# mrvollger/rustybam

Measured on AMD Instinct MI355X. Metric: CIGAR-ops/s, liftover over 100 kb sliding windows (whole pass, inputs resident in HBM), higher is better.
Workload: dtype u32

## Files before the change

### include/rustybam_amd.h

```cpp
#ifndef RUSTYBAM_AMD_H
#define RUSTYBAM_AMD_H

#include <stddef.h>
#include <stdint.h>

#ifdef __cplusplus
extern "C" {
#endif

#define RB_ABI_VERSION 1

enum rb_op { RB_OP_M = 0, RB_OP_I = 1, RB_OP_D = 2, RB_OP_N = 3, RB_OP_S = 4, RB_OP_H = 5, RB_OP_P = 6, RB_OP_EQ = 7, RB_OP_X = 8,
             RB_OP_CONT = 14  };

typedef enum rb_error {
    RB_OK = 0,
    RB_E_INVALID = -1,
    RB_E_NO_DEVICE = -2,
    RB_E_HIP = -3,
    RB_E_CAPACITY = -4,
    RB_E_NOMEM = -5
} rb_error;

typedef enum rb_status {
// ... 51 lines not shown
} rb_norm_row;

typedef struct rb_hit_row {
    uint32_t rec, win;
    uint16_t status, flags;
    uint32_t out_n;
    uint64_t t_st, t_en, q_st, q_en;
    uint32_t nmatch, aln_len;
    uint64_t out_off;
} rb_hit_row;

typedef struct rb_pair_row {
    uint64_t split_idx;
    int32_t split_score;
    uint32_t status;
    uint64_t t_st[2], t_en[2], q_st[2], q_en[2];
    uint32_t nmatch[2], aln_len[2];
    uint64_t out_off[2];
    uint32_t out_n[2];
    uint64_t _pad;
} rb_pair_row;

typedef struct rb_counters {
    uint64_t n_hits;
    uint64_t out_ops_needed;
    uint64_t out_ops_used;
    uint64_t n_generic;
    uint32_t overflow;
    uint32_t phase[5];
    uint32_t brk_scratch_short;
    uint32_t redo_two_walk;
} rb_counters;

enum { RB_TEXT_OK = 0, RB_TEXT_BAD = 1 , RB_TEXT_TOO_LONG = 2 ,
       RB_TEXT_UNUSUAL = 3  };

typedef struct rb_batch_view {
    uint64_t n_rec, n_ops;
    const uint32_t *ops;
    const uint64_t *op_off;
    const uint64_t *t_st, *t_en, *q_st, *q_en;
    const uint8_t *strand;
    const uint32_t *contig;
} rb_batch_view;

typedef struct rb_windows_view {
    uint64_t n_win;
    const uint32_t *contig;
    const uint64_t *st, *en;
} rb_windows_view;

typedef struct rb_ctx rb_ctx;
typedef struct rb_plan rb_plan;

int rb_abi_version(void);
int rb_device_count(void);
int rb_ctx_create(int device, void *hip_stream, rb_ctx **out);
void rb_ctx_destroy(rb_ctx *ctx);
const char *rb_ctx_last_error(const rb_ctx *ctx);
int rb_ctx_sync(rb_ctx *ctx);
void *rb_ctx_stream(rb_ctx *ctx);
int rb_ctx_set_timing(rb_ctx *ctx, int enabled);
int rb_ctx_get_timing(rb_ctx *ctx, double *ms_out, int cap, int *n_out);

int rb_dev_alloc(rb_ctx *ctx, size_t bytes, void **dev_ptr);
int rb_dev_free(rb_ctx *ctx, void *dev_ptr);
int rb_dev_alloc_mode(rb_ctx *ctx, const void *dev_ptr);
int rb_dev_release(rb_ctx *ctx, void *dev_ptr);
int rb_dev_cache_trim(rb_ctx *ctx, uint64_t keep_bytes);
int rb_dev_alloc_stats(rb_ctx *ctx, uint64_t out[5]);
int rb_dev_upload(rb_ctx *ctx, void *dev_dst, const void *host_src, size_t bytes);
int rb_dev_download(rb_ctx *ctx, void *host_dst, const void *dev_src, size_t bytes);
int rb_dev_memset(rb_ctx *ctx, void *dev_dst, int value, size_t bytes);

int rb_dev_scan_records(rb_ctx *ctx, const rb_batch_view *batch, rb_reduce_row *reduce_rows, rb_norm_row *norm_rows);
int rb_ctx_scan_route(rb_ctx *ctx, uint64_t out[2]);

int rb_plan_create(rb_ctx *ctx, uint64_t n_rec, const uint64_t *op_off_host, const uint32_t *contig_host,
                   uint64_t n_win, const uint32_t *w_contig_host, const uint64_t *w_st_host, const uint64_t *w_en_host,
                   rb_plan **out);
void rb_plan_destroy(rb_plan *plan);
int64_t rb_plan_tiles_host(uint64_t n_rec, const uint64_t *op_off_host, uint64_t short_max, uint32_t *sched_out, uint32_t *tiles_out,
                           uint64_t tiles_cap, uint64_t *n_long_out);
size_t rb_plan_workspace_bytes(const rb_plan *plan, uint64_t rows_cap);
size_t rb_plan_diag_stamps_offset(const rb_plan *plan, uint64_t rows_cap);
uint64_t rb_plan_out_capacity(const rb_plan *plan, int for_break);

int rb_dev_liftover(rb_ctx *ctx, const rb_plan *plan, const rb_batch_view *batch, const rb_norm_row *norm_rows,
                    int bsearch_policy, void *workspace, rb_hit_row *rows, uint64_t rows_cap, uint32_t *out_ops,
                    uint64_t out_cap, rb_counters *counters);

size_t rb_largest_scratch_bytes(uint64_t n_keys);
int rb_dev_largest(rb_ctx *ctx, const rb_hit_row *rows, uint64_t n_rows, const uint32_t *win_key, const uint32_t *rec_key,
                   uint64_t n_keys, uint64_t *sel, uint64_t *out, void *scratch);

int rb_dev_break(rb_ctx *ctx, const rb_plan *plan, const rb_batch_view *batch, const rb_norm_row *norm_rows,
                 uint32_t max_size, int bsearch_policy, void *workspace, rb_hit_row *rows, uint64_t rows_cap,
                 uint32_t *out_ops, uint64_t out_cap, rb_counters *counters);

int rb_dev_swap(rb_ctx *ctx, const rb_batch_view *batch, uint32_t *out_ops);

enum { RB_TRIM_IN_PLACE = 256 };
int rb_dev_overlap_split(rb_ctx *ctx, const rb_batch_view *batch, const rb_norm_row *norm_rows, uint64_t n_pairs,
                         const uint32_t *left, const uint32_t *right, const uint64_t *pair_out_off, int match_score,
                         int diff_score, int indel_score, int bsearch_policy, rb_pair_row *rows, uint32_t *out_ops);

int rb_dev_trim_reserve(rb_ctx *ctx, uint64_t n_pairs);

int rb_dev_apply_pairs(rb_ctx *ctx, uint64_t n_pairs, const uint32_t *left, const uint32_t *right, const rb_pair_row *rows,
                       uint64_t *op_off, rb_norm_row *norm_rows);

typedef struct rb_trim_pass {
    uint64_t n_pairs, n_deferred, ops_end;
    uint32_t bad_status, _pad;
    uint64_t _reserved[4];
} rb_trim_pass;
size_t rb_trim_select_scratch_bytes(uint64_t n_groups);
int rb_dev_trim_select(rb_ctx *ctx, uint64_t n_rec, uint64_t n_groups, const uint32_t *order, const uint64_t *grp_off,
                       const rb_norm_row *norm_rows, uint64_t out_base, uint8_t *contained, uint32_t *left, uint32_t *right,
                       uint64_t *pair_out_off, rb_trim_pass *pass, void *scratch);
int rb_dev_trim_check(rb_ctx *ctx, uint64_t n_pairs, const rb_pair_row *rows, rb_trim_pass *pass);
int rb_dev_gather_records(rb_ctx *ctx, uint64_t n_rec, const uint32_t *ops, const uint64_t *op_off, const rb_norm_row *norm_rows,
                          uint64_t *new_op_off, uint32_t *new_ops, void *scratch);

int rb_host_scan_records(rb_ctx *ctx, uint64_t n_rec, const uint32_t *ops, const uint64_t *op_off,
                         const uint64_t *t_st, const uint64_t *t_en, const uint64_t *q_st, const uint64_t *q_en,
                         const uint8_t *strand, rb_reduce_row *reduce_rows, rb_norm_row *norm_rows);
int rb_host_liftover(rb_ctx *ctx, uint64_t n_rec, const uint32_t *ops, const uint64_t *op_off, const uint64_t *t_st,
                     const uint64_t *t_en, const uint64_t *q_st, const uint64_t *q_en, const uint8_t *strand,
                     const uint32_t *contig, uint64_t n_win, const uint32_t *w_contig, const uint64_t *w_st,
                     const uint64_t *w_en, int bsearch_policy, rb_norm_row *norm_rows_out ,
                     rb_hit_row **rows, uint64_t *n_rows, uint32_t **out_ops, uint64_t *n_out, rb_counters *counters);
int rb_host_break(rb_ctx *ctx, uint64_t n_rec, const uint32_t *ops, const uint64_t *op_off, const uint64_t *t_st,
                  const uint64_t *t_en, const uint64_t *q_st, const uint64_t *q_en, const uint8_t *strand,
                  uint32_t max_size, int bsearch_policy, rb_norm_row *norm_rows_out, rb_hit_row **rows,
                  uint64_t *n_rows, uint32_t **out_ops, uint64_t *n_out, rb_counters *counters);
int rb_host_swap(rb_ctx *ctx, uint64_t n_rec, const uint32_t *ops, const uint64_t *op_off, const uint8_t *strand,
                 uint32_t *out_ops);
int rb_host_overlap_split(rb_ctx *ctx, uint64_t n_rec, const uint32_t *ops, const uint64_t *op_off, const uint64_t *t_st,
                          const uint64_t *t_en, const uint64_t *q_st, const uint64_t *q_en, const uint8_t *strand,
                          uint64_t n_pairs, const uint32_t *left, const uint32_t *right, int match_score, int diff_score,
                          int indel_score, int bsearch_policy, rb_pair_row *rows, uint32_t **out_ops, uint64_t *n_out);
void rb_host_free(void *p);

size_t rb_text_scratch_bytes(uint64_t n);
int rb_dev_parse_cigars(rb_ctx *ctx, const uint8_t *text, const uint64_t *text_off, const uint64_t *text_end, uint64_t n_rec,
                        uint64_t *op_off, uint32_t *ops, uint64_t ops_cap, uint8_t *status, void *scratch);
int rb_dev_format_cigars(rb_ctx *ctx, const uint32_t *ops, const uint32_t *ops_alt, uint64_t n_items, const uint64_t *first,
                         const uint32_t *count, const uint32_t *first_len, const uint32_t *last_len, uint64_t *text_off, uint8_t *text,
                         uint64_t text_cap, void *scratch);
int rb_host_parse_cigars(rb_ctx *ctx, const uint8_t *text, const uint64_t *text_off, const uint64_t *text_end, uint64_t n_rec,
                         uint64_t *op_off, uint32_t **ops, uint8_t *status);
int rb_host_format_cigars(rb_ctx *ctx, const uint32_t *ops, uint64_t n_ops, uint64_t n_items, const uint64_t *first, const uint32_t *count,
                          const uint32_t *first_len, const uint32_t *last_len, uint64_t *text_off, uint8_t **text);
int rb_host_liftover_text(rb_ctx *ctx, uint64_t n_rec, const uint8_t *text, uint64_t text_bytes, const uint64_t *cig_off,
                          const uint64_t *cig_end, const uint64_t *t_st, const uint64_t *t_en, const uint64_t *q_st, const uint64_t *q_en,
                          const uint8_t *strand, const uint32_t *contig, uint64_t n_win, const uint32_t *w_contig, const uint64_t *w_st,
                          const uint64_t *w_en, int bsearch_policy, uint8_t *cig_status, rb_reduce_row *reduce_out, rb_norm_row *norm_out,
                          rb_hit_row **rows, uint64_t *n_rows, uint64_t **row_text_off, uint8_t **row_text, rb_counters *counters);
int rb_host_liftover_largest_text(rb_ctx *ctx, uint64_t n_rec, const uint8_t *text, uint64_t text_bytes, const uint64_t *cig_off,
                                  const uint64_t *cig_end, const uint64_t *t_st, const uint64_t *t_en, const uint64_t *q_st, const uint64_t *q_en,
                                  const uint8_t *strand, const uint32_t *contig, uint64_t n_win, const uint32_t *w_contig, const uint64_t *w_st,
                                  const uint64_t *w_en, int bsearch_policy, uint8_t *cig_status, rb_reduce_row *reduce_out, rb_norm_row *norm_out,
                                  rb_hit_row **rows, uint64_t *n_rows, uint64_t **row_text_off, uint8_t **row_text, rb_counters *counters,
                                  const uint32_t *win_key, uint64_t n_keys, uint32_t inside_key, int *declined);
int rb_host_break_text(rb_ctx *ctx, uint64_t n_rec, const uint8_t *text, uint64_t text_bytes, const uint64_t *cig_off,
// ... 52 lines not shown
```

### rustybam_amd/capi.py

```python
import ctypes as C
import os
import sys
import re

import numpy as np

HERE = os.path.dirname(os.path.abspath(__file__))
ROOT = os.path.dirname(HERE)
HEADER = os.path.join(ROOT, "include", "rustybam_amd.h")

BSEARCH_MODERN, BSEARCH_LEGACY, LIFT_EARLY_EXIT, LIFT_DESCRIPTORS, LIFT_FUSED_SCAN = 0, 1, 16, 32, 64
TRIM_IN_PLACE = 256
LIFT_OP_STARTS = 1 << 20
BREAK_ONE_WALK = 128
HIT_INSIDE, HIT_GENERIC, HIT_DESCRIPTOR = 1, 2, 4
NF_COVERED = 0x80000000
RD_OK, RD_FILTERED, RD_BAD_CIGAR, RD_SEQ_SHORT = 0, 1, 2, 3

REDUCE_DT = np.dtype(
    [("t_bases", "<u8"), ("q_bases", "<u8"), ("nmatch", "<u4"), ("aln_len", "<u4"), ("equal", "<u4"),
     ("diff", "<u4"), ("ins", "<u4"), ("del", "<u4"), ("matches", "<u4"), ("ins_events", "<u4"),
     ("del_events", "<u4"), ("id_by_all", "<f4"), ("id_by_events", "<f4"), ("id_by_matches", "<f4"),
     ("status", "<u4"), ("flags", "<u4")])
NORM_DT = np.dtype(
# ... 397 lines not shown
        end = None if text_end is None else _arr(text_end, np.uint64)
        op_off = np.zeros(n + 1, np.uint64)
        status = np.zeros(max(n, 1), np.uint8)
        out = C.c_void_p()
        self._chk(self.L.rb_host_parse_cigars(self.ctx, _p(text), _p(text_off), _p(end) if end is not None else None,
                                              C.c_uint64(n), _p(op_off), C.byref(out), _p(status)), "rb_host_parse_cigars")
        n_ops = int(op_off[n])
        if n_ops:
            ops = np.frombuffer((C.c_char * (n_ops * 4)).from_address(out.value), dtype=np.uint32).copy()
        else:
            ops = np.zeros(0, np.uint32)
        self.L.rb_host_free(out)
        return op_off, ops, status[:n]

    def format_cigars(self, ops, first, count, first_len=None, last_len=None):
        ops, first, count = _arr(ops, np.uint32), _arr(first, np.uint64), _arr(count, np.uint32)
        n = len(first)
        fl = None if first_len is None else _arr(first_len, np.uint32)
        ll = None if last_len is None else _arr(last_len, np.uint32)
        toff = np.zeros(n + 1, np.uint64)
        out = C.c_void_p()
        src = np.concatenate([ops, np.zeros(4, np.uint32)])
        self._chk(self.L.rb_host_format_cigars(self.ctx, _p(src), C.c_uint64(len(ops)), C.c_uint64(n), _p(first), _p(count),
                                               _p(fl) if fl is not None else None, _p(ll) if ll is not None else None, _p(toff),
                                               C.byref(out)), "rb_host_format_cigars")
        nb = int(toff[n])
        text = bytes((C.c_char * nb).from_address(out.value)) if nb else b""
        self.L.rb_host_free(out)
        return toff, text


    def nucfreq_workspace_bytes(self, n_reads, n_regions, n_pos):
        f = self.L.rb_nucfreq_workspace_bytes
        f.restype = C.c_size_t
        return int(f(C.c_uint64(n_reads), C.c_uint64(n_regions), C.c_uint64(n_pos)))

    def dev_nucfreq(self, n_reads, ops, op_off, seq, seq_off, l_seq, tid, pos, flag, n_regions, rg_tid, rg_st, rg_en, out_off, n_pos,
                    counts, status, counters, ws, ws_bytes):
        class View(C.Structure):
            _fields_ = [("n_reads", C.c_uint64), ("ops", C.c_void_p), ("op_off", C.c_void_p), ("seq", C.c_void_p), ("seq_off", C.c_void_p),
                        ("l_seq", C.c_void_p), ("tid", C.c_void_p), ("pos", C.c_void_p), ("flag", C.c_void_p)]
        v = View(n_reads, ops, op_off, seq, seq_off, l_seq, tid, pos, flag)
        self._chk(self.L.rb_dev_nucfreq(self.ctx, C.byref(v), C.c_uint64(n_regions), C.c_void_p(rg_tid), C.c_void_p(rg_st), C.c_void_p(rg_en),
                                        C.c_void_p(out_off), C.c_uint64(n_pos), C.c_void_p(counts), C.c_void_p(status), C.c_void_p(counters),
                                        C.c_void_p(ws), C.c_size_t(ws_bytes)), "rb_dev_nucfreq")

    def nucfreq(self, tid, pos, flag, op_off, ops, l_seq, seq_off, seq, rg_tid, rg_st, rg_en):
        tid, pos, flag = _arr(tid, np.int32), _arr(pos, np.int64), _arr(flag, np.uint32)
        op_off, ops = _arr(op_off, np.uint64), np.concatenate([_arr(ops, np.uint32), np.zeros(4, np.uint32)])
        l_seq, seq_off = _arr(l_seq, np.uint32), _arr(seq_off, np.uint64)
        seq = np.concatenate([_arr(seq, np.uint8), np.zeros(32, np.uint8)])
        rg_tid, rg_st, rg_en = _arr(rg_tid, np.int32), _arr(rg_st, np.uint64), _arr(rg_en, np.uint64)
        n, nr = len(tid), len(rg_tid)
        n_pos = int((rg_en.astype(np.int64) - rg_st.astype(np.int64)).sum()) if nr else 0

        class View(C.Structure):
            _fields_ = [("n_reads", C.c_uint64), ("ops", C.c_void_p), ("op_off", C.c_void_p), ("seq", C.c_void_p), ("seq_off", C.c_void_p),
                        ("l_seq", C.c_void_p), ("tid", C.c_void_p), ("pos", C.c_void_p), ("flag", C.c_void_p)]
        v = View(n, ops.ctypes.data, op_off.ctypes.data, seq.ctypes.data, seq_off.ctypes.data, l_seq.ctypes.data, tid.ctypes.data,
                 pos.ctypes.data, flag.ctypes.data)
        counts = np.zeros((max(n_pos, 1), 4), np.uint32)
        status = np.zeros(max(n, 1), np.uint32)
        ctr = np.zeros(6, np.uint64)
        self._chk(self.L.rb_host_nucfreq(self.ctx, C.byref(v), C.c_uint64(nr), _p(rg_tid), _p(rg_st), _p(rg_en), _p(counts), _p(status),
                                         _p(ctr)), "rb_host_nucfreq")
        return counts[:n_pos], status[:n], dict(max_depth=int(ctr[0]), n_covered=int(ctr[1]), n_bad=int(ctr[2]), unsorted=int(ctr[3]),
                                                    n_dropped=int(ctr[4]), cap_overflow=int(ctr[5]))


def synth_n_ops(seed, first_record, n_rec, lo, hi):
    L = lib()
    return np.array([L.rb_synth_n_ops(seed, first_record + i, lo, hi) for i in range(n_rec)], dtype=np.uint64)


def synth_fill_ops_host(seed, first_record, op_off):
    L = lib()
    op_off = _arr(op_off, np.uint64)
    ops = np.zeros(int(op_off[-1]), np.uint32)
    L.rb_synth_fill_ops_host(C.c_uint64(seed), C.c_uint64(first_record), C.c_uint64(len(op_off) - 1), _p(op_off),
                             _p(ops))
    return ops


class DevBuf:

    def __init__(self, eng, torch, n, dtype, device=None, placed_tries=1, score=None):
        self.eng, self.n, self.dtype = eng, int(n), dtype
        self.item = torch.empty(0, dtype=dtype).element_size()
        self.placement = None

        def take():
            if placed_tries > 1:
                ptr, ms, kept = eng.dev_alloc_placed(max(self.n * self.item, 256), placed_tries, score)
                self.placement = {("launch_ms" if score else "sweep_ms"): ms, "kept": kept}
                return ptr
            return eng.dev_alloc(max(self.n * self.item, 256))
        try:
            self.ptr = take()
        except Exception:
            torch.cuda.empty_cache()
            self.ptr = take()
        self.chunked = eng.L.rb_dev_alloc_mode(eng.ctx, C.c_void_p(self.ptr)) == 1
        self.__cuda_array_interface__ = {"shape": (self.n * self.item,), "typestr": "|u1", "data": (self.ptr, False), "version": 3}
        try:
            self.t = torch.as_tensor(self, device=device if device is not None else "cuda").view(dtype)
            if device is not None and self.t.device != torch.device(device):
                raise RuntimeError(f"the buffer was taken for {self.t.device}, not {device}")
        except Exception:
            self.t = None
            eng.dev_free(self.ptr)
            self.ptr = 0
            raise

    def free(self):
        if self.ptr:
            self.t = None
            self.eng.dev_free(self.ptr)
            self.ptr = 0

    def release(self):
        if self.ptr:
            self.t = None
            self.eng.dev_release(self.ptr)
            self.ptr = 0
```

### rustybam_amd/csrc/capi.hip

```cpp
#include <hip/hip_runtime.h>
#include <sys/mman.h>

#include <algorithm>
#include <cstdarg>
#include <cstdio>
#include <cstdlib>
#include <cstring>
#include <ctime>
#include <numeric>
#include <string>
#include <thread>
#include <vector>
#include <chrono>
#include <map>
#include <mutex>

#include "../../include/rustybam_amd.h"
#include "rb_lift.h"
#include "rb_trim.h"
#include "rb_launch.h"

#ifndef RB_SCAN_ROWS_MEAN_MAX
#define RB_SCAN_ROWS_MEAN_MAX 1536
#endif
#ifndef RB_SHORT_MAX_DEFAULT
#define RB_SHORT_MAX_DEFAULT 2048
#endif

#define RB_MAX_ARENA 256

#define RB_TIMING_RING 256
__global__ __launch_bounds__(256) void rb_k_fill_bytes(uint8_t *dst, uint32_t v4, size_t n) {
    const uintptr_t a = (uintptr_t)dst;
    const size_t head = n < 16 ? n : (size_t)((16 - (a & 15)) & 15);
    const size_t body = (n - head) / 16;
    const size_t tail0 = head + body * 16;
    const size_t i = (size_t)blockIdx.x * blockDim.x + threadIdx.x, stride = (size_t)gridDim.x * blockDim.x;
    for (size_t k = i; k < body; k += stride) *reinterpret_cast<uint4 *>(dst + head + k * 16) = make_uint4(v4, v4, v4, v4);
    if (i < head) dst[i] = (uint8_t)v4;
    if (i < n - tail0) dst[tail0 + i] = (uint8_t)v4;
}
extern "C" hipError_t rb_fill_async(void *dst, int value, size_t bytes, hipStream_t stream) {
    if (!bytes) return hipSuccess;
    const uint32_t b = (uint32_t)value & 255u, v4 = b | (b << 8) | (b << 16) | (b << 24);
    const size_t groups = bytes / 16 + 1;
    const unsigned blocks = (unsigned)std::min<size_t>((groups + 255) / 256, 65536);
    hipLaunchKernelGGL(rb_k_fill_bytes, dim3(blocks ? blocks : 1), dim3(256), 0, stream, (uint8_t *)dst, v4, bytes);
    return hipGetLastError();
}

struct rb_ctx {
    int device = -1;
    hipStream_t stream = nullptr;
    bool own_stream = false;
    std::string err;
    bool timing = false;
    std::vector<hipEvent_t> ev_a, ev_b;
    uint64_t timed_calls = 0;
    void *trim_scratch = nullptr;
    uint32_t trim_scratch_blocks = 0;
    void *trim_pend = nullptr;
    uint64_t trim_pend_cap = 0;
    void *scan_list = nullptr;
    uint64_t scan_list_cap = 0;
    uint64_t scan_rows_n = 0;
    void *pin[2] = {nullptr, nullptr};
    hipEvent_t pin_ev[2] = {nullptr, nullptr};
    bool pin_busy[2] = {false, false};
    unsigned pin_next = 0;
    uint64_t alloc_fallbacks = 0;
    struct cached_buf { void *p; size_t bytes; bool placed; };
    std::vector<cached_buf> cache;
    size_t cache_bytes = 0;
};
#define RB_PIN_CHUNK ((size_t)32 << 20)
#define RB_PIN_MIN ((size_t)8 << 20)

struct rb_plan {
    rb_ctx *ctx = nullptr;
    uint64_t n_rec = 0, n_win = 0, n_ops = 0;
    uint32_t n_contig = 0;
    uint32_t depth = 0;
    uint32_t *sched = nullptr, *slot_of = nullptr, *canon_pos = nullptr, *w_orig = nullptr, *ident = nullptr;
    uint64_t *w_st = nullptr, *w_en = nullptr, *wo_st = nullptr, *wo_en = nullptr, *cw_off = nullptr;
    uint8_t *cw_mono = nullptr;
    uint32_t *tiles = nullptr;
    uint32_t n_tiles = 0, stream_end = 0;
};

static int fail(rb_ctx *ctx, int code, const char *fmt, ...) {
    if (ctx) {
        char buf[512];
        va_list ap;
        va_start(ap, fmt);
        vsnprintf(buf, sizeof buf, fmt, ap);
        va_end(ap);
        ctx->err = buf;
    }
    return code;
}
#define HIPCHK(ctx, call)                                                                             \
    do {                                                                                              \
        hipError_t e_ = (call);                                                                       \
        if (e_ != hipSuccess) return fail((ctx), RB_E_HIP, "%s: %s", #call, hipGetErrorString(e_)); \
    } while (0)

extern "C" int rb_abi_version(void) { return RB_ABI_VERSION; }

extern "C" int rb_device_count(void) {
    int n = 0;
    if (hipGetDeviceCount(&n) != hipSuccess) return 0;
    return n;
}

extern "C" int rb_ctx_create(int device, void *hip_stream, rb_ctx **out) {
    if (!out) return RB_E_INVALID;
    *out = nullptr;
    int n = 0;
    if (hipGetDeviceCount(&n) != hipSuccess || n <= 0 || device < 0 || device >= n) return RB_E_NO_DEVICE;
    hipDeviceProp_t prop;
    if (hipGetDeviceProperties(&prop, device) != hipSuccess) return RB_E_NO_DEVICE;
    if (strncmp(prop.gcnArchName, "gfx950", 6) != 0) {
        fprintf(stderr, "rustybam_amd: device %d is %s; this library only carries gfx950 (MI355X) code objects\n", device, prop.gcnArchName);
        return RB_E_NO_DEVICE;
    }
    if (hipSetDevice(device) != hipSuccess) return RB_E_NO_DEVICE;
    rb_ctx *c = new rb_ctx();
    c->device = device;
    if (hip_stream) {
        c->stream = (hipStream_t)hip_stream;
    } else {
        if (hipStreamCreateWithFlags(&c->stream, hipStreamNonBlocking) != hipSuccess) {
            delete c;
            return RB_E_HIP;
        }
        c->own_stream = true;
    }
    *out = c;
    return RB_OK;
}
extern "C" void rb_ctx_destroy(rb_ctx *ctx) {
    if (!ctx) return;
    for (auto e : ctx->ev_a) hipEventDestroy(e);
    for (auto e : ctx->ev_b) hipEventDestroy(e);
    for (int k = 0; k < 2; k++) {
        if (ctx->pin[k]) hipHostFree(ctx->pin[k]);
        if (ctx->pin_ev[k]) hipEventDestroy(ctx->pin_ev[k]);
    }
    if (ctx->trim_scratch) hipFree(ctx->trim_scratch);
    if (ctx->trim_pend) hipFree(ctx->trim_pend);
    if (ctx->scan_list) hipFree(ctx->scan_list);
    (void)rb_dev_cache_trim(ctx, 0);
    if (ctx->own_stream) hipStreamDestroy(ctx->stream);
    delete ctx;
}
extern "C" const char *rb_ctx_last_error(const rb_ctx *ctx) { return ctx ? ctx->err.c_str() : "no context"; }
extern "C" int rb_ctx_sync(rb_ctx *ctx) {
    if (!ctx) return RB_E_INVALID;
    HIPCHK(ctx, hipStreamSynchronize(ctx->stream));
    return RB_OK;
}
extern "C" void *rb_ctx_stream(rb_ctx *ctx) { return ctx ? (void *)ctx->stream : nullptr; }

extern "C" int rb_ctx_set_timing(rb_ctx *ctx, int enabled) {
    if (!ctx) return RB_E_INVALID;
    if (enabled && ctx->ev_a.empty()) {
        ctx->ev_a.resize(RB_TIMING_RING);
        ctx->ev_b.resize(RB_TIMING_RING);
        for (int i = 0; i < RB_TIMING_RING; i++) {
            HIPCHK(ctx, hipEventCreate(&ctx->ev_a[i]));
            HIPCHK(ctx, hipEventCreate(&ctx->ev_b[i]));
        }
    }
    ctx->timing = enabled != 0;
    ctx->timed_calls = 0;
    return RB_OK;
}
extern "C" int rb_ctx_get_timing(rb_ctx *ctx, double *ms_out, int cap, int *n_out) {
    if (!ctx || !ms_out || !n_out) return RB_E_INVALID;
    HIPCHK(ctx, hipStreamSynchronize(ctx->stream));
    const uint64_t have = ctx->timed_calls < RB_TIMING_RING ? ctx->timed_calls : RB_TIMING_RING;
    int n = 0;
    for (uint64_t k = 0; k < have && n < cap; k++) {
        const uint64_t call = ctx->timed_calls - have + k;
        const size_t slot = (size_t)(call % RB_TIMING_RING);
        float ms = 0;
        HIPCHK(ctx, hipEventElapsedTime(&ms, ctx->ev_a[slot], ctx->ev_b[slot]));
        ms_out[n++] = ms;
    }
    *n_out = n;
    return RB_OK;
}

struct rb_vmm_alloc {
    size_t bytes, chunk;
    std::vector<hipMemGenericAllocationHandle_t> handles;
    bool placed = false;
};
static std::map<void *, rb_vmm_alloc> g_vmm;
static std::mutex g_vmm_mu;
static size_t g_va_live = 0, g_va_retired = 0;
static std::map<void *, size_t> g_asked;
static size_t rb_va_cap() {
    const char *e = getenv("RB_ALLOC_VA_CAP_GB");
    return (size_t)(e ? strtoull(e, nullptr, 10) : 32768ull) << 30;
}
static int rb_free_vmm(void *p, int device, hipError_t *err) {
    std::lock_guard<std::mutex> lk(g_vmm_mu);
    auto it = g_vmm.find(p);
    if (it == g_vmm.end()) return 0;
    hipError_t first = hipSuccess;
// ... 316 lines not shown
}

extern "C" int rb_ctx_scan_route(rb_ctx *ctx, uint64_t out[2]) {
    if (!ctx || !out) return RB_E_INVALID;
    out[0] = out[1] = 0;
    if (!ctx->scan_rows_n) return RB_OK;
    unsigned long long n_listed = 0;
    HIPCHK(ctx, hipSetDevice(ctx->device));
    HIPCHK(ctx, hipMemcpyAsync(&n_listed, ctx->scan_list, sizeof n_listed, hipMemcpyDeviceToHost, ctx->stream));
    HIPCHK(ctx, hipStreamSynchronize(ctx->stream));
    out[0] = ctx->scan_rows_n - n_listed;
    out[1] = n_listed;
    return RB_OK;
}

template <typename T>
static int upload_vec(rb_ctx *ctx, const std::vector<T> &v, T **dev) {
    int rc = rb_dev_alloc(ctx, v.size() * sizeof(T) + 16, (void **)dev);
    if (rc) return rc;
    if (!v.empty()) {
        rc = rb_dev_upload(ctx, *dev, v.data(), v.size() * sizeof(T));
        if (rc) return rc;
    }
    return RB_OK;
}

static void rb_cut_tiles(uint64_t n_rec, const uint64_t *op_off, uint64_t short_max, std::vector<uint32_t> &sched, std::vector<uint32_t> &tiles,
                         uint64_t *n_long_out) {
    tiles.clear();
    *n_long_out = 0;
    short_max = std::min<uint64_t>(short_max, rb_tile_max_ops());
    if (short_max < 8 || !n_rec) return;
    const uint64_t max_ops = rb_tile_max_ops(), max_rec = rb_tile_max_records();
    std::vector<uint32_t> t2;
    uint64_t first = 0, cnt = 0, ops = 0, n_long = 0, n_tiled = 0;
    bool tiny = false;
    auto close = [&]() {
        if (cnt) t2.push_back((uint32_t)first | (tiny ? 0x80000000u : 0u)), t2.push_back((uint32_t)cnt), n_tiled += tiny ? 0 : cnt;
        cnt = 0, ops = 0;
    };
    for (uint64_t r = 0; r < n_rec; r++) {
        const uint64_t n = op_off[r + 1] - op_off[r];
        if (n > short_max) {
            close();
            n_long++;
            continue;
        }
        const bool t = n < 8;
        if (cnt && (t != tiny || cnt >= max_rec || (!t && ops + n > max_ops))) close();
        if (!cnt) first = r, tiny = t;
        cnt++, ops += n;
    }
    close();
    if (n_tiled == 0) return;
    std::vector<uint32_t> s2(n_rec);
    uint64_t a = 0, b = n_long;
    for (uint64_t w = 0; w < n_rec; w++)
        if (op_off[(uint64_t)sched[w] + 1] - op_off[sched[w]] > short_max) s2[a++] = sched[w];
    std::vector<uint32_t> slot_short(n_rec, 0);
    for (uint64_t r = 0; r < n_rec; r++)
        if (op_off[r + 1] - op_off[r] <= short_max) slot_short[r] = (uint32_t)b, s2[b++] = (uint32_t)r;
    sched.swap(s2);
    tiles.reserve(t2.size() / 2 * 3);
    for (size_t t = 0; t + 1 < t2.size(); t += 2) tiles.push_back(t2[t]), tiles.push_back(t2[t + 1]), tiles.push_back(slot_short[t2[t] & 0x7FFFFFFFu]);
    *n_long_out = n_long;
}
extern "C" int64_t rb_plan_tiles_host(uint64_t n_rec, const uint64_t *op_off, uint64_t short_max, uint32_t *sched_out, uint32_t *tiles_out,
                                      uint64_t tiles_cap, uint64_t *n_long_out) {
    if (n_rec && (!op_off || !sched_out)) return -1;
    if (n_rec >= 0xFFFFFFFFull) return -1;
    std::vector<uint32_t> sched(n_rec), tiles;
    std::iota(sched.begin(), sched.end(), 0u);
    std::stable_sort(sched.begin(), sched.end(), [&](uint32_t x, uint32_t y) { return op_off[(uint64_t)x + 1] - op_off[x] > op_off[(uint64_t)y + 1] - op_off[y]; });
    uint64_t n_long = 0;
    rb_cut_tiles(n_rec, op_off, short_max ? short_max : RB_SHORT_MAX_DEFAULT, sched, tiles, &n_long);
    for (uint64_t i = 0; i < n_rec; i++) sched_out[i] = sched[i];
    const uint64_t nt = tiles.size() / 3;
    for (uint64_t t = 0; t < nt && t < tiles_cap && tiles_out; t++)
        for (int k = 0; k < 3; k++) tiles_out[3 * t + k] = tiles[3 * t + k];
    if (n_long_out) *n_long_out = tiles.empty() ? n_rec : n_long;
    return (int64_t)nt;
}

extern "C" int rb_plan_create(rb_ctx *ctx, uint64_t n_rec, const uint64_t *op_off, const uint32_t *contig, uint64_t n_win,
                              const uint32_t *w_contig, const uint64_t *w_st, const uint64_t *w_en, rb_plan **out) {
    if (!ctx || !out || (n_rec && (!op_off || !contig))) return RB_E_INVALID;
    if (n_rec >= 0xFFFFFFFFull || n_win >= 0xFFFFFFFFull) return fail(ctx, RB_E_INVALID, "too many records/windows for one batch");
    HIPCHK(ctx, hipSetDevice(ctx->device));
    rb_plan *pl = new rb_plan();
    pl->ctx = ctx;
    pl->n_rec = n_rec;
    pl->n_win = n_win;
    uint32_t maxc = 0;
    for (uint64_t i = 0; i < n_rec; i++) maxc = std::max(maxc, contig[i]);
    for (uint64_t i = 0; i < n_win; i++) maxc = std::max(maxc, w_contig[i]);
    const uint32_t n_contig = (n_rec || n_win) ? maxc + 1 : 0;
    pl->n_contig = n_contig;
    std::vector<uint32_t> canon_pos(n_rec);
    {
        std::vector<uint64_t> rank(n_contig, UINT64_MAX);
        uint64_t nr = 0;
        for (uint64_t i = 0; i < n_rec; i++)
            if (rank[contig[i]] == UINT64_MAX) rank[contig[i]] = nr++;
        std::vector<uint64_t> start(nr + 1, 0);
        for (uint64_t i = 0; i < n_rec; i++) start[rank[contig[i]] + 1]++;
        for (uint64_t k = 0; k < nr; k++) start[k + 1] += start[k];
        for (uint64_t i = 0; i < n_rec; i++) canon_pos[i] = (uint32_t)start[rank[contig[i]]]++;
    }
    std::vector<uint32_t> sched(n_rec), ident(n_rec);
    std::iota(ident.begin(), ident.end(), 0u);
    {
        uint64_t max_len = 0;
        std::vector<uint64_t> key(n_rec);
        for (uint64_t i = 0; i < n_rec; i++) key[i] = op_off[i + 1] - op_off[i], max_len = std::max(max_len, key[i]);
        int passes = 0;
        while (passes < 4 && (max_len >> (16 * passes)) != 0) passes++;
        std::vector<uint32_t> a(ident), b(n_rec);
        std::vector<uint64_t> cnt(65537);
        for (int ps = 0; ps < passes; ps++) {
            std::fill(cnt.begin(), cnt.end(), 0);
            const int sh = 16 * ps;
            for (uint64_t i = 0; i < n_rec; i++) cnt[(0xFFFFu - (uint32_t)((key[i] >> sh) & 0xFFFFu)) + 1]++;
            for (int k = 0; k < 65536; k++) cnt[k + 1] += cnt[k];
            for (uint64_t i = 0; i < n_rec; i++) {
                const uint32_t r = a[i];
                b[cnt[0xFFFFu - (uint32_t)((key[r] >> sh) & 0xFFFFu)]++] = r;
            }
            a.swap(b);
        }
        sched = a;
    }
    std::vector<uint64_t> cw_off(n_contig + 1, 0), g_st(n_win), g_en(n_win), o_st(n_win), o_en(n_win);
    std::vector<uint32_t> g_orig(n_win);
    std::vector<uint8_t> mono(n_contig ? n_contig : 1, 1);
    for (uint64_t i = 0; i < n_win; i++) cw_off[w_contig[i] + 1]++;
    for (uint32_t c = 0; c < n_contig; c++) cw_off[c + 1] += cw_off[c];
    {
        std::vector<uint64_t> cur(cw_off.begin(), cw_off.end() - (n_contig ? 1 : 0));
        for (uint64_t i = 0; i < n_win; i++) {
            const uint64_t d = cur[w_contig[i]]++;
            g_st[d] = w_st[i];
            g_en[d] = w_en[i];
            g_orig[d] = (uint32_t)i;
            o_st[i] = w_st[i];
            o_en[i] = w_en[i];
        }
    }
    for (uint32_t c = 0; c < n_contig; c++)
        for (uint64_t i = cw_off[c] + 1; i < cw_off[c + 1]; i++)
            if (g_st[i] < g_st[i - 1] || g_en[i] < g_en[i - 1]) mono[c] = 0;
    pl->n_ops = n_rec ? op_off[n_rec] : 0;
    for (uint32_t c = 0; c < n_contig; c++) {
        if (!mono[c]) continue;
        uint64_t lo = cw_off[c];
        for (uint64_t i = cw_off[c]; i < cw_off[c + 1]; i++) {
            while (lo < i && g_en[lo] < g_st[i]) lo++;
            pl->depth = std::max<uint32_t>(pl->depth, (uint32_t)std::min<uint64_t>(i - lo + 1, 1u << 20));
        }
    }
    std::vector<uint32_t> tiles;
    pl->stream_end = (uint32_t)n_rec;
    {
        const char *e = getenv("RB_TILE");
        const bool on = !(e && !strcmp(e, "0"));
        uint64_t short_max = RB_SHORT_MAX_DEFAULT;
        if (const char *m = getenv("RB_SHORT_MAX")) short_max = strtoull(m, nullptr, 10);
        if (on && n_rec) {
            uint64_t n_long = 0;
            rb_cut_tiles(n_rec, op_off, short_max, sched, tiles, &n_long);
            if (!tiles.empty()) pl->stream_end = (uint32_t)n_long;
        }
        pl->n_tiles = (uint32_t)(tiles.size() / 3);
    }
    int rc = RB_OK;
    std::vector<uint32_t> slot_of(n_rec);
    for (uint64_t w = 0; w < n_rec; w++) slot_of[sched[w]] = (uint32_t)w;
    if (!rc) rc = upload_vec(ctx, sched, &pl->sched);
    if (!rc) rc = upload_vec(ctx, slot_of, &pl->slot_of);
    if (!rc) rc = upload_vec(ctx, ident, &pl->ident);
    if (!rc) rc = upload_vec(ctx, canon_pos, &pl->canon_pos);
    if (!rc) rc = upload_vec(ctx, g_st, &pl->w_st);
    if (!rc) rc = upload_vec(ctx, g_en, &pl->w_en);
    if (!rc) rc = upload_vec(ctx, g_orig, &pl->w_orig);
    if (!rc) rc = upload_vec(ctx, o_st, &pl->wo_st);
    if (!rc) rc = upload_vec(ctx, o_en, &pl->wo_en);
    if (!rc) rc = upload_vec(ctx, cw_off, &pl->cw_off);
    if (!rc) rc = upload_vec(ctx, mono, &pl->cw_mono);
    if (!rc && pl->n_tiles) rc = upload_vec(ctx, tiles, &pl->tiles);
    if (!rc && hipStreamSynchronize(ctx->stream) != hipSuccess) rc = fail(ctx, RB_E_HIP, "plan upload: %s", hipGetErrorString(hipGetLastError()));
    if (rc) {
        rb_plan_destroy(pl);
        return rc;
    }
    *out = pl;
    return RB_OK;
}
extern "C" void rb_plan_destroy(rb_plan *pl) {
    if (!pl) return;
    void *ptrs[] = {pl->sched, pl->slot_of, pl->ident, pl->canon_pos, pl->w_st, pl->w_en, pl->w_orig, pl->wo_st, pl->wo_en, pl->cw_off, pl->cw_mono, pl->tiles};
    for (void *q : ptrs)
        if (q) (void)rb_dev_free(pl->ctx, q);
    delete pl;
}

struct ws_layout {
    size_t hit_off, win_lo, block_sums, arena, pend_count, pend_list, jobs, gen_list, x_st, x_en, bp_tmp, bp_off, bp_cur, brk_rows, copy_count, copy_list, decl_count, decl_list, gen_cp, diag_stamps, fb_count, fb_list, starts_bad, total;
};
static bool rb_no_gen_cp() {
    static const bool v = getenv("RB_DEBUG_NO_GEN_CP") != nullptr;
    return v;
}
static ws_layout ws_of(uint64_t n_rec, uint64_t rows_cap, uint64_t n_ops) {
    ws_layout w;
    size_t o = 0;
    auto take = [&](size_t bytes) {
        size_t at = o;
        o += (bytes + 255) & ~(size_t)255;
        return at;
    };
    w.hit_off = take((n_rec + 2) * 8);
    w.win_lo = take((n_rec + 2) * 4);
    w.block_sums = take(rb_scan_block_sums_count(n_rec) * 8);
    w.arena = take((size_t)RB_MAX_ARENA * RB_ARENA_STRIDE * 8);
    w.pend_count = take(256);
    w.pend_list = take((n_rec + 1) * 4);
    w.jobs = take((n_rec + 1) * sizeof(rb_job));
    w.gen_list = take((rows_cap + 1) * 4);
    w.x_st = take((rows_cap + 1) * 8);
    w.x_en = take((rows_cap + 1) * 8);
    w.bp_tmp = take((rows_cap + 1) * 8);
    w.bp_off = take((n_rec + 1) * 8);
    w.bp_cur = take((size_t)RB_MAX_ARENA * 128);
    w.brk_rows = take((rows_cap + 1) * sizeof(rb_hit_row));
    w.copy_count = take(256);
    w.copy_list = take((rows_cap + 1) * 16);
    w.decl_count = take(256);
    w.decl_list = take((n_rec + 1) * 4);
    w.gen_cp = take(rb_no_gen_cp() ? 256 : (size_t)(n_ops / RB_GCP + n_rec + 2) * sizeof(uint4));
    w.diag_stamps = take((n_rec + 1) * 4);
    w.fb_count = take(256);
    w.fb_list = take((n_rec + 1) * 4);
    w.starts_bad = take(256);
    w.total = o;
    return w;
}
extern "C" size_t rb_plan_workspace_bytes(const rb_plan *plan, uint64_t rows_cap) {
    if (!plan) return 0;
    return ws_of(plan->n_rec, rows_cap, plan->n_ops).total;
}
extern "C" size_t rb_plan_diag_stamps_offset(const rb_plan *plan, uint64_t rows_cap) {
    if (!plan) return 0;
    return ws_of(plan->n_rec, rows_cap, plan->n_ops).diag_stamps;
// ... 1332 lines not shown
```

Baseline: 527.4 billion.

## Route single-record tiles into the long-record stream interleaved by length

Tiles that hold only one short record are removed from the tiled path and sent to the per-record streaming path instead. They are interleaved in groups of four among the long records, and slot indices for the remaining tiles are remapped. If no multi-record tiles remain, tiling is dropped entirely. The rerouting only happens when there are enough long records to fill the GPU (CU count x 4 SIMDs x 4 waves). The aim is to cut the waste of lonely tiles that occupy a whole workgroup, at the cost of changing load balance between the two paths.

Result: no change. 524.1 billion (-0.6%).

```diff
diff --git a/include/rustybam_amd.h b/include/rustybam_amd.h
--- a/include/rustybam_amd.h
+++ b/include/rustybam_amd.h
@@ -157,6 +157,8 @@
 void rb_plan_destroy(rb_plan *plan);
 int64_t rb_plan_tiles_host(uint64_t n_rec, const uint64_t *op_off_host, uint64_t short_max, uint32_t *sched_out, uint32_t *tiles_out,
                            uint64_t tiles_cap, uint64_t *n_long_out);
+int64_t rb_plan_route_host(uint64_t n_rec, const uint64_t *op_off_host, uint64_t short_max, uint64_t min_long, uint32_t *sched_out,
+                           uint32_t *tiles_out, uint64_t tiles_cap, uint64_t *stream_end_out);
 size_t rb_plan_workspace_bytes(const rb_plan *plan, uint64_t rows_cap);
 size_t rb_plan_diag_stamps_offset(const rb_plan *plan, uint64_t rows_cap);
 uint64_t rb_plan_out_capacity(const rb_plan *plan, int for_break);
diff --git a/rustybam_amd/capi.py b/rustybam_amd/capi.py
--- a/rustybam_amd/capi.py
+++ b/rustybam_amd/capi.py
@@ -503,6 +503,23 @@
     return ops
 
 
+def plan_route_host(n_ops, short_max=0, min_long=1):
+    L = lib()
+    L.rb_plan_route_host.restype = C.c_int64
+    n_ops = _arr(n_ops, np.uint64)
+    n = len(n_ops)
+    off = np.zeros(n + 1, np.uint64)
+    off[1:] = np.cumsum(n_ops)
+    sched = np.zeros(max(n, 1), np.uint32)
+    tiles = np.zeros(3 * max(n, 1), np.uint32)
+    stream_end = C.c_uint64(0)
+    nt = L.rb_plan_route_host(C.c_uint64(n), _p(off), C.c_uint64(short_max), C.c_uint64(min_long), _p(sched), _p(tiles), C.c_uint64(n),
+                              C.byref(stream_end))
+    if nt < 0:
+        raise RbError("rb_plan_route_host: bad arguments")
+    return sched[:n], tiles[: 3 * nt].reshape(-1, 3), int(stream_end.value)
+
+
 class DevBuf:
 
     def __init__(self, eng, torch, n, dtype, device=None, placed_tries=1, score=None):
diff --git a/rustybam_amd/csrc/capi.hip b/rustybam_amd/csrc/capi.hip
--- a/rustybam_amd/csrc/capi.hip
+++ b/rustybam_amd/csrc/capi.hip
@@ -51,6 +51,7 @@
 
 struct rb_ctx {
     int device = -1;
+    uint32_t n_cu = 0;
     hipStream_t stream = nullptr;
     bool own_stream = false;
     std::string err;
@@ -127,6 +128,7 @@
     if (hipSetDevice(device) != hipSuccess) return RB_E_NO_DEVICE;
     rb_ctx *c = new rb_ctx();
     c->device = device;
+    c->n_cu = (uint32_t)std::max(prop.multiProcessorCount, 1);
     if (hip_stream) {
         c->stream = (hipStream_t)hip_stream;
     } else {
@@ -609,6 +611,71 @@
     return (int64_t)nt;
 }
 
+#define RB_LIFT_WAVES_PER_SIMD 4u
+static void rb_route_lonely(uint64_t n_rec, const uint64_t *op_off, uint64_t min_long, std::vector<uint32_t> &sched, std::vector<uint32_t> &tiles,
+                            uint64_t *stream_end) {
+    const uint64_t n_long = *stream_end;
+    if (tiles.empty() || n_long == 0 || n_long < min_long) return;
+    auto len = [&](uint32_t r) { return op_off[(uint64_t)r + 1] - op_off[r]; };
+    std::vector<uint32_t> routed, kept;
+    std::vector<uint8_t> is_routed(n_rec, 0);
+    bool any_tile = false;
+    for (size_t t = 0; t + 2 < tiles.size(); t += 3) {
+        if (!(tiles[t] >> 31) && tiles[t + 1] == 1) {
+            routed.push_back(tiles[t]), is_routed[tiles[t]] = 1;
+            continue;
+        }
+        any_tile |= !(tiles[t] >> 31);
+        kept.insert(kept.end(), tiles.begin() + t, tiles.begin() + t + 3);
+    }
+    if (routed.empty()) return;
+    if (!any_tile) {
+        tiles.clear();
+        std::iota(sched.begin(), sched.end(), 0u);
+        std::stable_sort(sched.begin(), sched.end(), [&](uint32_t x, uint32_t y) { return len(x) > len(y); });
+        *stream_end = n_rec;
+        return;
+    }
+    std::stable_sort(routed.begin(), routed.end(), [&](uint32_t x, uint32_t y) { return len(x) > len(y); });
+    std::vector<uint32_t> s2;
+    s2.reserve(n_rec);
+    {
+        const uint64_t F = n_long / 4, G = routed.size() / 4;
+        uint64_t g = 0;
+        for (uint64_t b = 0; b <= F; b++) {
+            for (; g < G && (g + 1) * F / (G + 1) == b; g++) s2.insert(s2.end(), routed.begin() + 4 * g, routed.begin() + 4 * g + 4);
+            if (b < F) s2.insert(s2.end(), sched.begin() + 4 * b, sched.begin() + 4 * b + 4);
+        }
+        s2.insert(s2.end(), sched.begin() + 4 * F, sched.begin() + n_long);
+        s2.insert(s2.end(), routed.begin() + 4 * G, routed.end());
+    }
+    const uint64_t head = s2.size();
+    std::vector<uint32_t> slot_of(n_rec, 0);
+    for (uint64_t w = n_long; w < n_rec; w++)
+        if (!is_routed[sched[w]]) slot_of[sched[w]] = (uint32_t)s2.size(), s2.push_back(sched[w]);
+    for (size_t t = 0; t + 2 < kept.size(); t += 3) kept[t + 2] = slot_of[kept[t] & 0x7FFFFFFFu];
+    sched.swap(s2);
+    tiles.swap(kept);
+    *stream_end = head;
+}
+extern "C" int64_t rb_plan_route_host(uint64_t n_rec, const uint64_t *op_off, uint64_t short_max, uint64_t min_long, uint32_t *sched_out,
+                                      uint32_t *tiles_out, uint64_t tiles_cap, uint64_t *stream_end_out) {
+    if (n_rec && (!op_off || !sched_out)) return -1;
+    if (n_rec >= 0xFFFFFFFFull) return -1;
+    std::vector<uint32_t> sched(n_rec), tiles;
+    std::iota(sched.begin(), sched.end(), 0u);
+    std::stable_sort(sched.begin(), sched.end(), [&](uint32_t x, uint32_t y) { return op_off[(uint64_t)x + 1] - op_off[x] > op_off[(uint64_t)y + 1] - op_off[y]; });
+    uint64_t stream_end = 0;
+    rb_cut_tiles(n_rec, op_off, short_max ? short_max : RB_SHORT_MAX_DEFAULT, sched, tiles, &stream_end);
+    rb_route_lonely(n_rec, op_off, min_long, sched, tiles, &stream_end);
+    for (uint64_t i = 0; i < n_rec; i++) sched_out[i] = sched[i];
+    const uint64_t nt = tiles.size() / 3;
+    for (uint64_t t = 0; t < nt && t < tiles_cap && tiles_out; t++)
+        for (int k = 0; k < 3; k++) tiles_out[3 * t + k] = tiles[3 * t + k];
+    if (stream_end_out) *stream_end_out = tiles.empty() ? n_rec : stream_end;
+    return (int64_t)nt;
+}
+
 extern "C" int rb_plan_create(rb_ctx *ctx, uint64_t n_rec, const uint64_t *op_off, const uint32_t *contig, uint64_t n_win,
                               const uint32_t *w_contig, const uint64_t *w_st, const uint64_t *w_en, rb_plan **out) {
     if (!ctx || !out || (n_rec && (!op_off || !contig))) return RB_E_INVALID;
@@ -692,9 +759,14 @@
         const bool on = !(e && !strcmp(e, "0"));
         uint64_t short_max = RB_SHORT_MAX_DEFAULT;
         if (const char *m = getenv("RB_SHORT_MAX")) short_max = strtoull(m, nullptr, 10);
+        const char *l = getenv("RB_LONELY");
+        const bool lonely = !(l && !strcmp(l, "0"));
+        uint64_t min_long = (uint64_t)ctx->n_cu * 4u * RB_LIFT_WAVES_PER_SIMD;
+        if (const char *m = getenv("RB_LONELY_MIN_LONG")) min_long = strtoull(m, nullptr, 10);
         if (on && n_rec) {
             uint64_t n_long = 0;
             rb_cut_tiles(n_rec, op_off, short_max, sched, tiles, &n_long);
+            if (lonely) rb_route_lonely(n_rec, op_off, min_long, sched, tiles, &n_long);
             if (!tiles.empty()) pl->stream_end = (uint32_t)n_long;
         }
         pl->n_tiles = (uint32_t)(tiles.size() / 3);
```
